# RaikoPipe/panda-gym

Hardware: AMD Instinct MI355X
Metric: aggregate env-steps/s, PandaReach 4096 envs @1 GPU; 1/2/4/8-GPU scaling (higher is better)
Workload: dtype f32; 1 GPU; PandaReach-v3 (ee control, sparse reward), 4096 envs per GPU, the reference's scene: table / plane contacts of the robot (BASELINE configs[1]); envs_per_gpu=4096, global_envs=4096, parallelism=env-sharded x1

## Files before the change

panda-gym_amd/csrc/pgx_api.cpp:

```cpp
#include <hip/hip_runtime.h>

#include <cmath>
#include <cstdarg>
#include <cstdio>
#include <cstdlib>
#include <cstring>
#include <string>
#include <vector>

#include "../../include/pgx.h"
#include "pgx_default_model.h"
#include "pgx_dev.h"
#include "pgx_model_consts.h"
#include "pgx_rows.h"

namespace {

thread_local std::string g_err;

int fail(int code, const char* fmt, ...) __attribute__((format(printf, 2, 3)));
int fail(int code, const char* fmt, ...) {
    char buf[512];
    va_list ap;
    va_start(ap, fmt);
// ... 10 lines not shown

void m3mul(const double* A, const double* B, double* C) {
    double t[9];
    for (int i = 0; i < 3; i++)
        for (int j = 0; j < 3; j++) t[i * 3 + j] = A[i * 3] * B[j] + A[i * 3 + 1] * B[3 + j] + A[i * 3 + 2] * B[6 + j];
    std::memcpy(C, t, sizeof t);
}
void m3v(const double* A, const double* v, double* o) {
    double t[3];
    for (int i = 0; i < 3; i++) t[i] = A[i * 3] * v[0] + A[i * 3 + 1] * v[1] + A[i * 3 + 2] * v[2];
    std::memcpy(o, t, sizeof t);
}

}

int pgx_set_error(int code, const char* msg) {
    g_err = msg;
    return code;
}

struct pgx_env {
    int device;
    PgxDevModel dm;
    PgxDevModel* dm_dev;
    PgxDevEnv de;
    PgxDevState ds;
    void* blob;
    size_t blob_bytes;
    std::vector<void*> snaps;
    uint64_t* pcg = nullptr;
    bool pcg_set = false;
    int man_pool = 0;
    const char* step_kernel = nullptr;
};

extern "C" {

const char* pgx_version(void) { return "pgx 0.1.0 (gfx950)"; }
const char* pgx_last_error(void) { return g_err.c_str(); }

int pgx_obs_dim(const pgx_config* c) {
    if (!c) return PGX_E_INVALID;
    if (c->task == PGX_TASK_REACH_AO) return 20 + 4 * PGX_AO_LINKS;
    return 6 + (c->block_gripper ? 0 : 1) + (c->task == PGX_TASK_REACH ? 0 : 12);
}
int pgx_action_dim(const pgx_config* c) {
    if (!c) return PGX_E_INVALID;
    return (c->control == PGX_CONTROL_EE ? 3 : 7) + (c->block_gripper ? 0 : 1);
}

static int check_compiled_tables(const PgxDevModel& dm) {
    auto same = [](const float* a, const float* b, int n, const char* what) -> int {
        for (int i = 0; i < n; i++)
            if (std::fabs(a[i] - b[i]) > 1e-6f * std::fmax(1.0f, std::fabs(b[i])))
                return fail(PGX_E_UNSUPPORTED, "model table %s[%d] = %g differs from the compiled robot (%g)", what,
                            i, (double)a[i], (double)b[i]);
        return PGX_OK;
    };
    int rc = 0;
    rc = rc ? rc : same(&dm.jp[0][0], &kJp[0][0], 21, "jp");
    rc = rc ? rc : same(&dm.jr[0][0], &kJr[0][0], 63, "jr");
    rc = rc ? rc : same(&dm.com[0][0], &kCom[0][0], 21, "com");
    rc = rc ? rc : same(dm.mass, kMass, 7, "mass");
    rc = rc ? rc : same(&dm.inertia[0][0], &kInertia[0][0], 18, "inertia");
    rc = rc ? rc : same(dm.i6c, kI6c, 6, "i6c");
    rc = rc ? rc : same(dm.i6own, kI6own, 6, "i6own");
// ... 294 lines not shown
        return fail(PGX_E_INVALID, "n_substeps must be in [1, 1000], got %d", cfg->params->n_substeps);
    pgx_env* h = new pgx_env();
    h->device = device;
    int rc = build_dev_model(cfg, &h->dm);
    if (rc) { delete h; return rc; }
#ifndef PGX_RUNTIME_MODEL
    {
        static_assert(sizeof(PgxDevModel) == 4 * PGX_DEV_MODEL_WORDS, "default model block size");
        const PgxDevModelWords& def = cfg->task == PGX_TASK_REACH_AO ? kDefModelAoWords : kDefModelArmWords;
        uint32_t got[PGX_DEV_MODEL_WORDS];
        std::memcpy(got, &h->dm, sizeof got);
        for (int i = 0; i < PGX_DEV_MODEL_WORDS; i++)
            if (got[i] != def.w[i]) {
                delete h;
                return fail(PGX_E_UNSUPPORTED,
                            "physics / robot parameters differ from the ones the kernels are compiled for "
                            "(constant block word %d: 0x%08x, compiled 0x%08x; tools/gen_default_model.py)",
                            i, got[i], def.w[i]);
            }
    }
#endif
    PgxDevEnv& e = h->de;
    e.pcg = nullptr;
    e.pcg_on = nullptr;
    e.perm_buf = nullptr;
    e.perm = nullptr;
    e.sort_mode = 0;
    if (const char* so = std::getenv("PGX_SORT_ENVS")) e.sort_mode = std::atoi(so) ? 1 : -1;
    e.sort_key = 1;
    if (const char* sk = std::getenv("PGX_SORT_KEY")) e.sort_key = std::atoi(sk) ? 1 : 0;
    e.sort_segs = 0;
    if (const char* sg = std::getenv("PGX_SORT_SEGS")) e.sort_segs = std::atoi(sg) == 1 ? 1 : 0;
    e.perm_segs = 1;
    e.task = cfg->task;
    e.control = cfg->control;
    e.reward = cfg->reward;
    e.n_envs = cfg->n_envs;
    e.max_episode_steps = cfg->max_episode_steps;
    e.block_gripper = cfg->block_gripper;
    e.obs_dim = pgx_obs_dim(cfg);
    e.action_dim = pgx_action_dim(cfg);
    e.seed = cfg->seed;
    e.env_id_offset = cfg->env_id_offset;
    e.distance_threshold = cfg->distance_threshold;
    for (int c = 0; c < 3; c++) { e.goal_low[c] = cfg->goal_low[c]; e.goal_high[c] = cfg->goal_high[c]; }
    for (int c = 0; c < 3; c++) {
        e.goal_offset[c] = cfg->goal_offset[c];
        e.obj_low[c] = cfg->obj_low[c];
        e.obj_high[c] = cfg->obj_high[c];
        e.obj_offset[c] = cfg->obj_offset[c];
    }
    e.goal_z_zero_prob = cfg->goal_z_zero_prob;
    e.contacts = cfg->contacts ? 1 : 0;
    e.full_manifold = cfg->contacts == PGX_CONTACTS_FULL ? 1 : 0;
    e.has_object = has_object;
    e.obj_half = (float)cfg->object_half;
    e.obj_inv_mass = e.has_object ? (float)(1.0 / cfg->object_mass) : 0.0f;
    e.obj_inv_inertia = e.has_object ? (float)(1.0 / cfg->object_inertia) : 0.0f;
    e.table_cx = (float)cfg->table_center[0];
    e.table_cy = (float)cfg->table_center[1];
    e.table_hx = (float)cfg->table_half[0];
    e.table_hy = (float)cfg->table_half[1];
    e.table_top = (float)(cfg->table_center[2] + cfg->table_half[2]);
    e.plane_z = (float)cfg->plane_z;
    e.table_hz = (float)cfg->table_half[2];
    e.ao = cfg->task == PGX_TASK_REACH_AO;
// ... 9 lines not shown
    }
    e.pgs_mode = 0;
    if (const char* pm = std::getenv("PGX_PGS_MODE")) e.pgs_mode = std::atoi(pm);
    e.n_substeps = cfg->params->n_substeps;
    e.wave_mode = 0;
    if (const char* wm = std::getenv("PGX_WAVES_PER_SIMD")) e.wave_mode = std::atoi(wm);
    const int wide_max = 8192;
    e.lanes_per_env = cfg->lanes_per_env ? cfg->lanes_per_env
                                         : ((cfg->n_envs <= wide_max || cfg->contacts) ? 16 : 1);
    if (const char* lpe = std::getenv("PGX_LANES_PER_ENV")) {
        const int v = std::atoi(lpe);
        if (v != 1 && v != 16) { delete h; return fail(PGX_E_INVALID, "PGX_LANES_PER_ENV must be 1 or 16, got %s", lpe); }
        e.lanes_per_env = v;
    }
    if (e.full_manifold && e.lanes_per_env != 16) {
        delete h;
        return fail(PGX_E_UNSUPPORTED, "PGX_CONTACTS_FULL needs the 16-lane layout (the one-lane kernels keep 4 robot points)");
    }

    rc = hip_check(hipSetDevice(device), "hipSetDevice");
    if (rc) { delete h; return rc; }
    const size_t N = (size_t)cfg->n_envs;
    auto align = [](size_t x) { return (x + 255) & ~(size_t)255; };
    const int man_pool = (e.full_manifold && (e.has_object || e.ao)) ? (e.has_object ? PGX_MANIFOLD_POOL
                                                                                     : PGX_MANIFOLD_POOL_AO) : 0;
    const size_t man_rows = man_pool ? 1 + (size_t)man_pool * PGX_MANIFOLD_POINT : 0;
    h->man_pool = man_pool;
    size_t off_goal = align(sizeof(PgxDevModel)), off_q = align(off_goal + 3 * N * 8), off_qd = align(off_q + PGX_NJ * N * 4),
           off_qc = align(off_qd + PGX_NJ * N * 4), off_obj = align(off_qc + PGX_NJ * N * 4), off_ct = align(off_obj + 13 * N * 4),
           off_ao = align(off_ct + 2 * PGX_CONTACT_SLOTS * N * 4),
           off_man = align(off_ao + (e.ao ? 4 * PGX_AO_OBSTACLES * N * 4 : 0)),
           off_el = align(off_man + man_rows * N * 4), off_ep = align(off_el + N * 4),
           off_err = align(off_ep + N * 4), off_perm = align(off_err + 4),
           total = align(off_perm + (e.full_manifold ? N * 4 + (N + 3) / 4 * 4 + (N / 256 + 1) * 13 * 4 : 0));
    rc = hip_check(hipMalloc(&h->blob, total), "hipMalloc(state)");
    if (rc) { delete h; return rc; }
    h->blob_bytes = total;
    char* b = (char*)h->blob;
    h->ds.goal = (double*)(b + off_goal);
    h->ds.q = (float*)(b + off_q);
    h->ds.qd = (float*)(b + off_qd);
    h->ds.qc = (float*)(b + off_qc);
    h->ds.object = (float*)(b + off_obj);
    h->ds.contacts = (float*)(b + off_ct);
    h->ds.obstacles = e.ao ? (float*)(b + off_ao) : nullptr;
    h->ds.man = man_pool ? (float*)(b + off_man) : nullptr;
    h->ds.elapsed = (int32_t*)(b + off_el);
    h->ds.episode = (uint32_t*)(b + off_ep);
    h->ds.errors = (uint32_t*)(b + off_err);
    if (e.full_manifold) e.perm_buf = (int32_t*)(b + off_perm);
    h->dm_dev = (PgxDevModel*)b;
    const size_t pcg_bytes = align(8 * PGX_PCG64_WORDS * N);
    const size_t geo_bytes = e.ao ? align(8 * PGX_AO_GEO_DOUBLES) : 0;
    rc = hip_check(hipMalloc((void**)&h->pcg, pcg_bytes + 256 + geo_bytes), "hipMalloc(rng streams)");
    if (rc) { h->pcg = nullptr; (void)hipFree(h->blob); delete h; return rc; }
    e.pcg = h->pcg;
    e.pcg_on = (const int32_t*)((char*)h->pcg + pcg_bytes);
    e.ao_geo = e.ao ? (const double*)((char*)h->pcg + pcg_bytes + 256) : nullptr;
    rc = hip_check(hipMemset(h->pcg, 0, pcg_bytes + 256), "hipMemset(rng streams)");
    if (!rc && e.ao) {
        double geo[PGX_AO_GEO_DOUBLES];
        ao_reset_geometry(cfg, geo);
        rc = hip_check(hipMemcpy((void*)e.ao_geo, geo, sizeof geo, hipMemcpyHostToDevice), "ReachAO geometry copy");
    }
    if (!rc) rc = hip_check(hipMemset(h->blob, 0, total), "hipMemset(state)");
    if (!rc) rc = hip_check(hipMemcpy(h->dm_dev, &h->dm, sizeof(PgxDevModel), hipMemcpyHostToDevice), "model copy");
    if (!rc && e.perm_buf) {
        std::vector<int32_t> ident(N);
        for (size_t k = 0; k < N; k++) ident[k] = (int32_t)k;
        rc = hip_check(hipMemcpy(e.perm_buf, ident.data(), N * 4, hipMemcpyHostToDevice), "env order init");
    }
    if (!rc) {
        PgxDevOut none;
        std::memset(&none, 0, sizeof none);
        rc = hip_check((hipError_t)pgx_launch_reset(h->dm_dev, h->de, h->ds, nullptr, nullptr, nullptr, none, nullptr),
                       "reset launch");
        if (!rc) rc = hip_check(hipMemset(h->ds.episode, 0, N * 4), "hipMemset(episode)");
        if (!rc) rc = hip_check(hipDeviceSynchronize(), "create sync");
    }
    if (rc) { (void)hipFree(h->pcg); (void)hipFree(h->blob); delete h; return rc; }
    *out = h;
    return PGX_OK;
}
// ... 22 lines not shown
    out->errors = h->ds.errors;
    out->robot_points = !h->de.contacts ? 0
                      : !h->de.full_manifold ? PGX_ROBOT_POINTS_ONE_LANE
                      : h->de.has_object ? PGX_ROBOT_POINTS : PGX_ROBOT_POINTS_ARM;
    out->env_order = h->de.perm_buf;
    out->manifolds = h->ds.man;
    out->manifold_pool = h->man_pool;
    return PGX_OK;
}

static PgxDevOut to_dev_out(const pgx_step_out* o) {
    PgxDevOut d;
    std::memset(&d, 0, sizeof d);
    if (!o) return d;
    d.obs = o->obs;
    d.ag = o->achieved_goal;
    d.dg = o->desired_goal;
    d.reward = o->reward;
    d.success = o->success;
    d.terminated = o->terminated;
    d.truncated = o->truncated;
    d.terminal_obs = o->terminal_obs;
    d.terminal_ag = o->terminal_achieved_goal;
    d.terminal_dg = o->terminal_desired_goal;
    d.task_truncated = o->task_truncated;
    return d;
}

int pgx_reset(pgx_handle h, const uint8_t* env_mask, const double* inject_goal, const double* inject_object,
              pgx_step_out* out, void* stream) {
    if (!h) return fail(PGX_E_INVALID, "null handle");
    if (inject_object && !h->de.has_object && !h->de.ao)
        return fail(PGX_E_INVALID, "object injection needs an object task (or ReachAO obstacles)");
    return hip_check((hipError_t)pgx_launch_reset(h->dm_dev, h->de, h->ds, env_mask, inject_goal, inject_object,
                                                  to_dev_out(out), stream),
                     "reset launch");
}

int pgx_step(pgx_handle h, const float* action, pgx_step_out* out, void* stream) {
    if (!h || !action) return fail(PGX_E_INVALID, "null argument");
    if (out && out->nonfinite && !h->de.nonfinite_guard) {
        const int rc = hip_check((hipError_t)pgx_launch_zero_flags(out->nonfinite, h->de.n_envs, stream), "flags launch");
        if (rc) return rc;
    }
    return hip_check((hipError_t)pgx_launch_step(h->dm_dev, h->de, h->ds, action, to_dev_out(out), stream,
                                                 &h->step_kernel, out ? out->nonfinite : nullptr),
                     "step launch");
}

const char* pgx_step_kernel(pgx_handle h) { return h ? h->step_kernel : nullptr; }

int pgx_sample_actions(pgx_handle h, float* action, uint64_t step, void* stream) {
    if (!h || !action) return fail(PGX_E_INVALID, "null argument");
    return hip_check((hipError_t)pgx_launch_sample_actions(h->de, action, step, stream), "sample launch");
}

int pgx_compute_reward(const float* ag, const float* dg, int64_t batch, int32_t reward_type, double thr, float* out,
                       void* stream) {
    if (batch < 0 || (batch > 0 && (!ag || !dg || !out))) return fail(PGX_E_INVALID, "bad arguments");
    if (reward_type != PGX_REWARD_SPARSE && reward_type != PGX_REWARD_DENSE && reward_type != PGX_REWARD_SPARSE_AO)
        return fail(PGX_E_INVALID, "reward_type %d", reward_type);
    return hip_check((hipError_t)pgx_launch_compute_reward(ag, dg, batch, reward_type, thr, out, stream),
                     "compute_reward launch");
}

int pgx_state_bytes(pgx_handle h, int64_t* nbytes) {
    if (!h || !nbytes) return fail(PGX_E_INVALID, "null argument");
    *nbytes = (int64_t)h->blob_bytes;
    return PGX_OK;
}

int pgx_save_state(pgx_handle h, void* dst, void* stream) {
    if (!h || !dst) return fail(PGX_E_INVALID, "null argument");
    return hip_check(hipMemcpyAsync(dst, h->blob, h->blob_bytes, hipMemcpyDeviceToDevice, (hipStream_t)stream),
                     "save_state copy");
}

int pgx_restore_state(pgx_handle h, const void* src, void* stream) {
    if (!h || !src) return fail(PGX_E_INVALID, "null argument");
    return hip_check(hipMemcpyAsync(h->blob, src, h->blob_bytes, hipMemcpyDeviceToDevice, (hipStream_t)stream),
                     "restore_state copy");
}

int pgx_snapshot(pgx_handle h, int32_t* state_id, void* stream) {
    if (!h || !state_id) return fail(PGX_E_INVALID, "null argument");
    *state_id = -1;
    size_t id = 0;
    while (id < h->snaps.size() && h->snaps[id]) id++;
    int rc = hip_check(hipSetDevice(h->device), "hipSetDevice");
    void* buf = nullptr;
    if (!rc) rc = hip_check(hipMalloc(&buf, h->blob_bytes), "hipMalloc(snapshot)");
    if (rc) return rc;
    rc = hip_check(hipMemcpyAsync(buf, h->blob, h->blob_bytes, hipMemcpyDeviceToDevice, (hipStream_t)stream),
                   "snapshot copy");
    if (rc) { (void)hipFree(buf); return rc; }
    if (id == h->snaps.size()) h->snaps.push_back(buf);
    else h->snaps[id] = buf;
    *state_id = (int32_t)id;
    return PGX_OK;
}

static bool snap_valid(pgx_handle h, int32_t id) {
    return id >= 0 && (size_t)id < h->snaps.size() && h->snaps[id] != nullptr;
}

int pgx_restore(pgx_handle h, int32_t state_id, void* stream) {
    if (!h) return fail(PGX_E_INVALID, "null handle");
    if (!snap_valid(h, state_id)) return fail(PGX_E_INVALID, "Couldn't restore state %d: no such saved state", state_id);
    return hip_check(hipMemcpyAsync(h->blob, h->snaps[state_id], h->blob_bytes, hipMemcpyDeviceToDevice,
                                    (hipStream_t)stream),
                     "restore copy");
}

int pgx_release(pgx_handle h, int32_t state_id) {
    if (!h) return fail(PGX_E_INVALID, "null handle");
    if (!snap_valid(h, state_id)) return fail(PGX_E_INVALID, "Couldn't remove state %d: no such saved state", state_id);
    int rc = hip_check(hipSetDevice(h->device), "hipSetDevice");
    if (!rc) rc = hip_check(hipDeviceSynchronize(), "release sync");
    if (!rc) rc = hip_check(hipFree(h->snaps[state_id]), "hipFree(snapshot)");
    h->snaps[state_id] = nullptr;
    return rc;
}

int pgx_set_rng_streams(pgx_handle h, const uint64_t* states, void* stream) {
    if (!h) return fail(PGX_E_INVALID, "null handle");
    int rc = hip_check(hipSetDevice(h->device), "hipSetDevice");
    if (rc) return rc;
    int32_t* on = const_cast<int32_t*>(h->de.pcg_on);
    if (states)
        rc = hip_check(hipMemcpyAsync(h->pcg, states, 8 * PGX_PCG64_WORDS * (size_t)h->de.n_envs, hipMemcpyDefault, (hipStream_t)stream),
                       "rng streams copy");
    if (!rc) rc = hip_check((hipError_t)pgx_launch_set_word(on, states ? 1 : 0, stream), "rng mode word");
    if (!rc) h->pcg_set = states != nullptr;
    return rc;
}

int pgx_get_rng_streams(pgx_handle h, uint64_t* states, void* stream) {
    if (!h || !states) return fail(PGX_E_INVALID, "null argument");
    if (!h->pcg_set) return fail(PGX_E_INVALID, "no PCG64 reset streams set (pgx_set_rng_streams)");
    return hip_check(hipMemcpyAsync(states, h->pcg, 8 * PGX_PCG64_WORDS * (size_t)h->de.n_envs, hipMemcpyDefault, (hipStream_t)stream),
                     "rng streams copy");
// ... 4 lines not shown
```

panda-gym_amd/csrc/pgx_dev.h:

```cpp
#pragma once
#include <stdint.h>

#define PGX_NJ 7
#define PGX_MAX_DAMP 4

struct PgxDevModel {
    float jp[PGX_NJ][3];
    float jr[PGX_NJ][9];
    float com[PGX_NJ][3];
    float mass[PGX_NJ];
    float inertia[PGX_NJ - 1][3];
    float i6c[6];
    float i6own[6];
    float dpos[PGX_MAX_DAMP][3];
    float dmass[PGX_MAX_DAMP];
    int32_t ndamp;
    float ee_pivot[3];
    float ee_rot[9];
    float ee_com[3];
    float lower[PGX_NJ], upper[PGX_NJ];
    float max_impulse[PGX_NJ];
    float dt, inv_dt;
    float gravity[3];
    float lin_damp, ang_damp, max_vel, residual_thr, erp, limit_max_imp, kp, kd;
// ... 13 lines not shown
struct PgxDevEnv {
    int32_t task, control, reward, n_envs;
    int32_t max_episode_steps, block_gripper, obs_dim, action_dim;
    uint64_t seed, env_id_offset;
    double distance_threshold;
    double goal_low[3], goal_high[3];
    double goal_offset[3], goal_z_zero_prob;
    double obj_low[3], obj_high[3], obj_offset[3];
    int32_t contacts, has_object;
    float obj_half, obj_inv_mass, obj_inv_inertia;
    float table_cx, table_cy, table_hx, table_hy, table_top, plane_z;
    float table_hz;
    int32_t ao;
    int32_t terminate_on_success;
    int32_t no_auto_reset;
    double collision_reward;
    double ao_ee[3];
    int32_t ao_ee_set;
    const double* ao_geo;
    int32_t lanes_per_env;
    int32_t pgs_mode;
    int32_t n_substeps;
    int32_t full_manifold;
    int32_t wave_mode;
    uint64_t* pcg;
    const int32_t* pcg_on;
    int32_t* perm_buf;
    int32_t sort_mode;
    int32_t sort_key;
    int32_t sort_segs;
    const int32_t* perm;
    int32_t perm_segs;
    int32_t nonfinite_guard;
};

struct PgxDevState {
    float* q;
    float* qd;
    float* qc;
    double* goal;
    float* object;
    float* contacts;
    float* obstacles;
    float* man;
    int32_t* elapsed;
    uint32_t* episode;
    uint32_t* errors;
};

struct PgxDevOut {
    float* obs;
    float* ag;
    float* dg;
    float* reward;
    uint8_t* success;
    uint8_t* terminated;
    uint8_t* truncated;
    float* terminal_obs;
    float* terminal_ag;
    float* terminal_dg;
    uint8_t* task_truncated;
};

int pgx_launch_step_arm(const PgxDevModel* m_device, const PgxDevEnv& e, const PgxDevState& s, const float* action,
                        const PgxDevOut& o, void* stream, const char** name, uint8_t* nonfinite);
int pgx_launch_step(const PgxDevModel* m_device, const PgxDevEnv& e, const PgxDevState& s, const float* action,
// ... 17 lines not shown
```

panda-gym_amd/csrc/pgx_kernels.hip:

```cpp
#include <hip/hip_runtime.h>
#include <math.h>
#include <stdint.h>

#include "../../include/pgx.h"
#include "pgx_default_model.h"
#include "pgx_common.h"
#include "pgx_dev.h"
#include "pgx_model_consts.h"
#include "pgx_rows.h"

#ifdef PGX_PROF
#define PGX_PROF_N 24
__device__ unsigned long long pgx_prof_counters[PGX_PROF_N];
#define PGX_PROF_WAVES 16384
__device__ unsigned long long pgx_prof_wave[PGX_PROF_WAVES][10];
extern "C" int pgx_prof_wave_read(unsigned long long* out, int n) {
    return (int)hipMemcpyFromSymbol(out, HIP_SYMBOL(pgx_prof_wave), sizeof(unsigned long long) * 10 * (size_t)n);
}
extern "C" int pgx_prof_read(unsigned long long* out, int clear) {
    hipError_t e = hipMemcpyFromSymbol(out, HIP_SYMBOL(pgx_prof_counters), sizeof(unsigned long long) * PGX_PROF_N);
    if (e == hipSuccess && clear) {
        unsigned long long z[PGX_PROF_N] = {0};
        e = hipMemcpyToSymbol(HIP_SYMBOL(pgx_prof_counters), z, sizeof z);
    }
// ... 3895 lines not shown
        if (t < AO_N - n_active) { L.aoC[pt][0][ln] = 99.9f; L.aoC[pt][1][ln] = 99.9f; L.aoC[pt][2][ln] = -99.9f; }
    }
    if (inject_goal) { goal[0] = inject_goal[0]; goal[1] = inject_goal[1]; goal[2] = inject_goal[2]; }
    if (inject_obst)
        for (int o = 0; o < AO_N; o++)
            for (int k = 0; k < 3; k++) L.aoC[o][k][ln] = (float)inject_obst[3 * o + k];
    if (rec && lead && !inject_goal && !inject_obst) pcg64_store(d.g, rec);
    return failed && !inject_obst;
}

template <class LT>
__device__ __forceinline__ void ao_load(const PgxDevState& s, int N, int i, LT& L, int ln) {
#pragma unroll
    for (int o = 0; o < AO_N; o++)
#pragma unroll
        for (int k = 0; k < 3; k++) L.aoC[o][k][ln] = s.obstacles[(3 * o + k) * N + i];
}
template <class LT>
__device__ __forceinline__ void ao_store(const PgxDevState& s, int N, int i, const LT& L, int ln) {
#pragma unroll
    for (int o = 0; o < AO_N; o++) {
#pragma unroll
        for (int k = 0; k < 3; k++) s.obstacles[(3 * o + k) * N + i] = L.aoC[o][k][ln];
        s.obstacles[(3 * AO_N + o) * N + i] = L.aoC[o][0][ln] < 50.0f ? 1.0f : 0.0f;
    }
}

__device__ __forceinline__ int xcd_block() {
    const int nb = gridDim.x, b = blockIdx.x;
    if (nb % 8) return b;
    return (b % 8) * (nb / 8) + b / 8;
}

template <int CONTROL, int OBJ, int CONT, int AO, int WIDE, int PART = 1, int GUARD = 0>
__device__ __forceinline__ void step_body(const PgxDevModel* __restrict__ mdev, const PgxDevEnv& e,
                                          const PgxDevState& s, const float* __restrict__ action, const PgxDevOut& o,
                                          uint8_t* nf_out = nullptr) {
    constexpr int FULL = WIDE == 2 ? 1 : 0;
    using LT = ContactLdsT<WIDE ? EPW : 64, WIDE ? OBJ : 1, FULL>;
    constexpr int CACHE_K = 2 * (CG + LT::RB);
    const int ln = WIDE ? (int)threadIdx.x / GW : (int)threadIdx.x;
    const int c = WIDE ? (int)threadIdx.x % GW : 0;
    const bool lead = c == 0;
    const int N = e.n_envs;
    const int slot = ((e.perm && e.perm_segs == 1) ? (int)blockIdx.x : xcd_block()) * (WIDE ? EPW : 64) + ln;
    if (slot >= N) return;
    const int i = e.perm ? e.perm[slot] : slot;
#ifdef PGX_CHECK_PERM
    if ((unsigned)i >= (unsigned)N) {
        printf("pgx: perm[%d] = %d outside [0, %d)\n", slot, i, N);
        __builtin_trap();
    }
#endif
    int ii = i;
    asm volatile("" : "+v"(ii));
    LT* L = nullptr;
    if constexpr (CONT) {
        __shared__ LT lds_buf;
        L = &lds_buf;
#ifdef PGX_LDS_POISON
        {
            float* w = reinterpret_cast<float*>(L);
            for (size_t t = threadIdx.x; t < sizeof(LT) / 4; t += blockDim.x) w[t] = __builtin_nanf("");
            __syncthreads();
        }
#endif
#pragma unroll
        for (int k = 0; k < (WIDE ? 0 : CG); k++) {
#pragma unroll
            for (int qq = 0; qq < 4; qq++) L->g0q[k][qq][ln] = make_float4(0.0f, 0.0f, 0.0f, 0.0f);
            L->g0n[k][0][ln] = 0.0f; L->g0n[k][1][ln] = 0.0f; L->g0n[k][2][ln] = 1.0f;
#pragma unroll
            for (int dir = 0; dir < 3; dir++)
#pragma unroll
                for (int qq = 0; qq < 6; qq++) L->g1q[k][dir][qq][ln] = make_float4(0.0f, 0.0f, 0.0f, 0.0f);
        }
    }
#ifdef PGX_PROF
    if (threadIdx.x < PGX_PROF_N) g_prof[threadIdx.x] = 0;
    g_prof_t = __builtin_amdgcn_s_memtime();
// ... 106 lines not shown
            if constexpr (AO) asm volatile("" : "+v"(cl), "+v"(esl));
            if (substep_g<OBJ, CONT, PART, AO, FULL>(mp, e, q, qd, tq, ob, L, esl, cl, lk, AO && st > 0)) {
                collided = true;
                break;
            }
        } else {
            substep<OBJ, CONT, AO>(mp, e, q, qd, tq, ob, L, ln);
        }
        if constexpr (PARK) qslot = st & 1;
        else {
#pragma unroll
            for (int j = 0; j < NJ; j++) qprev[j] = qstart[j];
        }
        if constexpr (AO && !WIDE) {
            ao_caps(*fresh(mp), q, *L, ln);
            if (ao_collided(e, *L, ln)) { collided = true; break; }
        }
    }
    if constexpr (AO && WIDE) {
        if (!collided) {
            ao_caps(*fresh(mp), q, *L, ln);
            collided = ao_collided_g(e, *L, ln, c);
        }
    }

    if constexpr (PARK) {
#pragma unroll
        for (int j = 0; j < NJ; j++) qprev[j] = lds_ld(&L->lqs[qslot][j][ln]);
    }
    int ie = i;
    if constexpr (AO) {
        int lnx = ln;
        asm volatile("" : "+v"(lnx));
        const int sl = ((e.perm && e.perm_segs == 1) ? (int)blockIdx.x : xcd_block()) * (WIDE ? EPW : 64) + lnx;
        ie = e.perm ? __hip_atomic_load(&e.perm[sl], __ATOMIC_RELAXED, __HIP_MEMORY_SCOPE_AGENT) : sl;
    }
    double goal[3];
#pragma unroll
    for (int c = 0; c < 3; c++) goal[c] = s.goal[c * N + (AO ? ie : ii)];
    V3 pos, vel;
    ee_state_cached(*fresh(mp), qprev, q, qd, pos, vel);
#ifdef PGX_NAN_TRAP
    if constexpr (!WIDE) {
        const float pv[6] = {pos.x, pos.y, pos.z, vel.x, vel.y, vel.z};
        PGX_TRAP(7, 0, pv, 6, m);
    }
#endif
    const int od = e.obs_dim;
    const V3 ag = OBJ ? ob.p : pos;
    double d = distance_f32_f64(ag, goal);
    bool succ = d < e.distance_threshold;
    float rew;
    if (AO) {
        rew = -1.0f + ((d + (collided ? 1.0 : 0.0)) < e.distance_threshold ? 1.0f : 0.0f);
        if (collided) rew += (float)e.collision_reward;
    } else {
        rew = e.reward == 0 ? -((d > e.distance_threshold) ? 1.0f : 0.0f) : -(float)d;
    }
    int el = s.elapsed[ie] + 1;
    uint32_t episode = s.episode[ie];
    bool trunc = (e.max_episode_steps > 0 && el >= e.max_episode_steps) || collided;
    bool term = e.terminate_on_success && succ;
    bool bad = false;
    if constexpr (GUARD) {
        if constexpr (AO) {
            if constexpr (WIDE) ao_link_obs_g(*L, ln, c);
            else ao_link_obs(*L, ln);
// ... 105 lines not shown
    if (o.dg) {
        o.dg[3 * (size_t)ie] = (float)goal[0]; o.dg[3 * (size_t)ie + 1] = (float)goal[1];
        o.dg[3 * (size_t)ie + 2] = (float)goal[2];
    }
    if constexpr (GUARD) {
        if (bad && !e.no_auto_reset) {
            if (o.terminal_obs) {
                if constexpr (AO) ao_write_obs(o.terminal_obs + (size_t)ie * od, pos, vel, q, qd, *L, ln);
                else write_obs<OBJ>(e, o.terminal_obs + (size_t)ie * od, pos, vel, ob);
            }
            if (o.terminal_ag) {
                o.terminal_ag[3 * (size_t)ie] = ag2.x; o.terminal_ag[3 * (size_t)ie + 1] = ag2.y;
                o.terminal_ag[3 * (size_t)ie + 2] = ag2.z;
            }
            if (o.terminal_dg) {
                o.terminal_dg[3 * (size_t)ie] = (float)goal[0]; o.terminal_dg[3 * (size_t)ie + 1] = (float)goal[1];
                o.terminal_dg[3 * (size_t)ie + 2] = (float)goal[2];
            }
        }
    }
#pragma unroll
    for (int j = 0; j < NJ; j++) {
        s.q[j * N + ie] = q[j];
        s.qd[j * N + ie] = qd[j];
        s.qc[j * N + ie] = qprev[j];
    }
#pragma unroll
    for (int c = 0; c < 3; c++) s.goal[c * N + ie] = goal[c];
    if (OBJ) store_obj(s, N, ie, ob);
    if constexpr (AO) ao_store(s, N, ie, *L, ln);
    if (CONT) {
#pragma unroll
        for (int k = 0; k < CACHE_K; k++) s.contacts[k * N + ie] = L->cache[k][ln];
    }
    s.elapsed[ie] = el;
    s.episode[ie] = episode;
#ifdef PGX_PROF
    PGX_PROF_MARK(6);
    if (threadIdx.x == 0) {
        for (int k = 0; k < PGX_PROF_N; k++) atomicAdd(&pgx_prof_counters[k], g_prof[k]);
        if (blockIdx.x < PGX_PROF_WAVES) {
            unsigned long long* w = pgx_prof_wave[blockIdx.x];
            w[0] = prof_t0; w[1] = g_prof_t; w[2] = g_prof[8]; w[3] = g_prof[10]; w[4] = g_prof[12]; w[5] = g_prof[13];
            w[6] = g_prof[7]; w[7] = g_prof[4]; w[8] = g_prof[1]; w[9] = g_prof[6];
        }
    }
#endif
}

template <int AO>
__device__ __forceinline__ void scene_from_model(PgxDevEnv& e, const PgxDevModel* mdev) {
    if constexpr (!AO) return;
    MRef m = *model_ptr<AO>(mdev);
    e.table_cx = m.table_cx; e.table_cy = m.table_cy; e.table_hx = m.table_hx; e.table_hy = m.table_hy;
    e.table_top = m.table_top; e.plane_z = m.plane_z; e.table_hz = m.table_hz;
}
template <int CONTROL, int OBJ, int CONT, int AO, int WIDE>
__global__ __launch_bounds__(64) void step_kernel(const PgxDevModel* __restrict__ mdev, PgxDevEnv e, PgxDevState s,
                                                  const float* __restrict__ action, PgxDevOut o) {
    scene_from_model<AO>(e, mdev);
    step_body<CONTROL, OBJ, CONT, AO, WIDE>(mdev, e, s, action, o);
}
template <int CONTROL, int OBJ, int CONT, int AO, int WIDE>
__global__ __launch_bounds__(64) __attribute__((amdgpu_waves_per_eu(2, 2))) void step_kernel_o2(
    const PgxDevModel* __restrict__ mdev, PgxDevEnv e, PgxDevState s, const float* __restrict__ action, PgxDevOut o) {
    scene_from_model<AO>(e, mdev);
// ... 80 lines not shown
    if (OBJ) store_obj(s, N, i, ob);
    if constexpr (AO) ao_store(s, N, i, *L, ln);
#pragma unroll
    for (int k = 0; k < CACHE_N; k++) s.contacts[k * N + i] = (k & 1) ? 0.0f : -1.0f;
    if (s.man) s.man[i] = 0.0f;
    s.elapsed[i] = 0;
    s.episode[i] = episode;
}

__global__ __launch_bounds__(256) void sample_actions_kernel(PgxDevEnv e, float* action, uint64_t step) {
    const int i = blockIdx.x * blockDim.x + threadIdx.x;
    if (i >= e.n_envs) return;
    const int A = e.action_dim;
    const uint64_t env = e.env_id_offset + (uint64_t)i;
    uint32_t o[4];
    for (int a = 0; a < A; a++) {
        if ((a & 3) == 0)
            philox((uint32_t)env, (uint32_t)(env >> 32), (uint32_t)step,
                   TAG_ACTION + ((uint32_t)(step >> 32) << 4) + (uint32_t)(a >> 2), (uint32_t)e.seed,
                   (uint32_t)(e.seed >> 32), o);
        uint32_t u = o[a & 3];
        action[(size_t)i * A + a] = (float)(u >> 8) * (1.0f / 16777216.0f) * 2.0f - 1.0f;
    }
}

__global__ __launch_bounds__(256) void compute_reward_kernel(const float* __restrict__ ag, const float* __restrict__ dg,
                                                             int64_t n, int32_t reward_type, float thr,
                                                             float* __restrict__ out) {
    for (int64_t i = blockIdx.x * (int64_t)blockDim.x + threadIdx.x; i < n; i += (int64_t)gridDim.x * blockDim.x) {
        out[i] = reward_f32(distance_f32_f32(ag + 3 * i, dg + 3 * i), reward_type, thr);
    }
}

constexpr int SORT_BINS = PGX_ROBOT_POINTS + 1;
constexpr int SORT_BLOCK = 256;
__global__ __launch_bounds__(SORT_BLOCK) void env_sort_keys_kernel(PgxDevState s, int N, int rb, int all, uint8_t* keys,
                                                                   int32_t* blk) {
    __shared__ int32_t wc[SORT_BLOCK / 64][SORT_BINS];
    const int i = blockIdx.x * SORT_BLOCK + threadIdx.x, lane = (int)__lane_id(), w = (int)threadIdx.x / 64;
    int key = -1;
    if (i < N) {
        key = 0;
        for (int r = 0; r < rb; r++) key += s.contacts[(size_t)(CACHE1 + 2 * r) * N + i] >= 0.0f ? 1 : 0;
        if (!all) key = key > CG ? key - CG : 0;
        keys[i] = (uint8_t)key;
    }
    for (int k = 0; k < SORT_BINS; k++) {
        const int c = __popcll(__ballot(key == k));
        if (lane == 0) wc[w][k] = c;
    }
    __syncthreads();
    if (threadIdx.x < SORT_BINS) {
        int c = 0;
        for (int ww = 0; ww < SORT_BLOCK / 64; ww++) c += wc[ww][threadIdx.x];
        blk[(size_t)blockIdx.x * SORT_BINS + threadIdx.x] = c;
    }
}
__global__ __launch_bounds__(SORT_BLOCK) void env_sort_scatter_kernel(int N, const uint8_t* keys, const int32_t* blk,
                                                                      int32_t* perm, int segs) {
    __shared__ int32_t base[SORT_BINS];
    __shared__ int32_t wc[SORT_BLOCK / 64][SORT_BINS];
    const int bps = (int)gridDim.x / segs, me = (int)blockIdx.x, sg = me / bps;
    const int b0 = sg * bps, nb = b0 + bps;
    const int i = me * SORT_BLOCK + threadIdx.x, lane = (int)__lane_id(), w = (int)threadIdx.x / 64;
    __shared__ int32_t red[SORT_BLOCK / 64][2][SORT_BINS];
    int tot[SORT_BINS], pre[SORT_BINS];
#pragma unroll
// ... 9 lines not shown
#pragma unroll
    for (int k = 0; k < SORT_BINS; k++) {
#pragma unroll
        for (int d = 32; d >= 1; d >>= 1) {
            tot[k] += __shfl_xor(tot[k], d);
            pre[k] += __shfl_xor(pre[k], d);
        }
        if (lane == 0) { red[w][0][k] = tot[k]; red[w][1][k] = pre[k]; }
    }
    __syncthreads();
    if (threadIdx.x < SORT_BINS) {
        const int k = threadIdx.x;
        int off = 0;
        for (int kk = SORT_BINS - 1; kk > k; kk--)
            for (int ww = 0; ww < SORT_BLOCK / 64; ww++) off += red[ww][0][kk];
        for (int ww = 0; ww < SORT_BLOCK / 64; ww++) off += red[ww][1][k];
        base[k] = off + sg * (N / segs);
    }
    const int key = i < N ? (int)keys[i] : -1;
    uint64_t mine_k = 0ull;
    for (int k = 0; k < SORT_BINS; k++) {
        const uint64_t m = __ballot(key == k);
        if (key == k) mine_k = m;
        if (lane == 0) wc[w][k] = __popcll(m);
    }
    __syncthreads();
    if (key >= 0) {
        int r = base[key] + __popcll(mine_k & ((1ull << lane) - 1ull));
        for (int ww = 0; ww < w; ww++) r += wc[ww][key];
        perm[r] = i;
    }
}

constexpr int SORT_SEG_MAX = 1024;
__global__ __launch_bounds__(SORT_SEG_MAX) void env_sort_segment_kernel(PgxDevState s, int N, int rb, int all,
                                                                        int32_t* perm) {
    __shared__ int32_t wc[SORT_SEG_MAX / 64][SORT_BINS];
    __shared__ int32_t base[SORT_BINS];
    const int S = (int)blockDim.x, t = (int)threadIdx.x, lane = (int)__lane_id(), w = t / 64, nw = (S + 63) / 64;
    const int i = (int)blockIdx.x * S + t;
    int key = 0;
    for (int r = 0; r < rb; r++) key += s.contacts[(size_t)(CACHE1 + 2 * r) * N + i] >= 0.0f ? 1 : 0;
    if (!all) key = key > CG ? key - CG : 0;
    uint64_t mine_k = 0ull;
    for (int k = 0; k < SORT_BINS; k++) {
        const uint64_t m = __ballot(key == k);
        if (key == k) mine_k = m;
        if (lane == 0) wc[w][k] = __popcll(m);
    }
    __syncthreads();
    if (t < SORT_BINS) {
        int off = 0;
        for (int kk = SORT_BINS - 1; kk > t; kk--)
            for (int ww = 0; ww < nw; ww++) off += wc[ww][kk];
        base[t] = off;
    }
    __syncthreads();
    int r = base[key] + __popcll(mine_k & ((1ull << lane) - 1ull));
    for (int ww = 0; ww < w; ww++) r += wc[ww][key];
    perm[(int)blockIdx.x * S + r] = i;
}

}

#ifndef PGX_TU
#define PGX_TU 0
#endif
// ... 13 lines not shown
        if (two) {                                                                                           \
            hipLaunchKernelGGL((step_kernel_o2_nf<C, O, K, A, W>), grid, block, 0, st, m, e, s, action, o, nf); \
            if (name) *name = PGX_KNAME(step_kernel_o2_nf, C, O, K, A, W);                                   \
        } else {                                                                                             \
            PGX_STEP(C, O, K, A, W);                                                                         \
        }                                                                                                    \
    } while (0)
#else
#define PGX_FN(f) f
#define PGX_STEP(C, O, K, A, W)                                                                   \
    do {                                                                                          \
        hipLaunchKernelGGL((step_kernel<C, O, K, A, W>), grid, block, 0, st, m, e, s, action, o); \
        if (name) *name = PGX_KNAME(step_kernel, C, O, K, A, W);                                  \
    } while (0)
#define PGX_STEP2(C, O, K, A, W)                                                                      \
    do {                                                                                              \
        if (two) {                                                                                    \
            hipLaunchKernelGGL((step_kernel_o2<C, O, K, A, W>), grid, block, 0, st, m, e, s, action, o); \
            if (name) *name = PGX_KNAME(step_kernel_o2, C, O, K, A, W);                                \
        } else {                                                                                      \
            PGX_STEP(C, O, K, A, W);                                                                  \
        }                                                                                             \
    } while (0)
#endif
#if PGX_TU != 3 && PGX_TU != 4
constexpr unsigned kSortMinWaves = 256u;
static PgxDevEnv sort_envs(const PgxDevEnv& e, const PgxDevState& s, hipStream_t st) {
    PgxDevEnv es = e;
    const int rb = e.has_object ? PGX_ROBOT_POINTS : PGX_ROBOT_POINTS_ARM;
    {
        const int segs = (e.sort_segs != 1 && e.n_envs % (8 * SORT_BLOCK) == 0) ? 8 : 1;
        const int S = e.n_envs / segs;
        if (S <= SORT_SEG_MAX && S > 0) {
            hipLaunchKernelGGL(env_sort_segment_kernel, dim3(segs), dim3(S), 0, st, s, e.n_envs, rb, e.sort_key,
                               e.perm_buf);
            es.perm = e.perm_buf;
            es.perm_segs = segs;
            return es;
        }
    }
    const int nb = (e.n_envs + SORT_BLOCK - 1) / SORT_BLOCK;
    uint8_t* keys = reinterpret_cast<uint8_t*>(e.perm_buf + e.n_envs);
    int32_t* blk = e.perm_buf + e.n_envs + (e.n_envs + 3) / 4;
    hipLaunchKernelGGL(env_sort_keys_kernel, dim3(nb), dim3(SORT_BLOCK), 0, st, s, e.n_envs, rb, e.sort_key, keys, blk);
    const int segs = (e.sort_segs != 1 && e.n_envs % (8 * SORT_BLOCK) == 0) ? 8 : 1;
    hipLaunchKernelGGL(env_sort_scatter_kernel, dim3(nb), dim3(SORT_BLOCK), 0, st, e.n_envs, (const uint8_t*)keys,
                       (const int32_t*)blk, e.perm_buf, segs);
    es.perm = e.perm_buf;
    es.perm_segs = segs;
    return es;
}
#endif
#if PGX_TU == 4 || PGX_TU == 0
int PGX_FN(pgx_launch_step_ao)(const PgxDevModel* m, const PgxDevEnv& e, const PgxDevState& s, const float* action,
                               const PgxDevOut& o, void* stream, const char** name, bool two, bool wide, uint8_t* nf) {
    hipStream_t st = (hipStream_t)stream;
    const int per_block = wide ? EPW : 64;
    dim3 block(64), grid((e.n_envs + per_block - 1) / per_block);
    if (wide && e.full_manifold) PGX_STEP2(1, 0, 1, 1, 2);
    else if (wide) PGX_STEP2(1, 0, 1, 1, 1);
    else PGX_STEP(1, 0, 1, 1, 0);
    return (int)hipGetLastError();
}
#endif
#if PGX_TU != 2 && PGX_TU != 3 && PGX_TU != 4
int PGX_FN(pgx_launch_step_arm)(const PgxDevModel* m, const PgxDevEnv& e, const PgxDevState& s, const float* action,
                                const PgxDevOut& o, void* stream, const char** name, uint8_t* nf) {
    hipStream_t st = (hipStream_t)stream;
    const int wide = e.lanes_per_env == GW;
    const int per_block = wide ? EPW : 64;
    dim3 block(64), grid((e.n_envs + per_block - 1) / per_block);
    const bool two = e.wave_mode == 2 || (e.wave_mode == 0 && wide && grid.x > 1024);
    if (wide && e.contacts && e.full_manifold) {
        PgxDevEnv es = e;
        es.perm = nullptr;
        if (e.perm_buf && (e.sort_mode == 1 || (e.sort_mode == 0 && grid.x >= kSortMinWaves))) es = sort_envs(e, s, st);
        const PgxDevEnv& e = es;
        if (e.control) PGX_STEP(1, 0, 1, 0, 2);
        else PGX_STEP2(0, 0, 1, 0, 2);
        return (int)hipGetLastError();
    }
    switch ((e.control * 4 + (e.contacts ? 1 : 0)) * 2 + wide) {
        case 0: PGX_STEP(0, 0, 0, 0, 0); break;
        case 1: PGX_STEP(0, 0, 0, 0, 1); break;
        case 2: PGX_STEP(0, 0, 1, 0, 0); break;
        case 3: PGX_STEP2(0, 0, 1, 0, 1); break;
        case 8: PGX_STEP(1, 0, 0, 0, 0); break;
        case 9: PGX_STEP(1, 0, 0, 0, 1); break;
        case 10: PGX_STEP(1, 0, 1, 0, 0); break;
        case 11: PGX_STEP(1, 0, 1, 0, 1); break;
        default: return (int)hipErrorInvalidValue;
    }
    return (int)hipGetLastError();
}
#endif
#if PGX_TU != 1 && PGX_TU != 3 && PGX_TU != 4
int PGX_FN(pgx_launch_step)(const PgxDevModel* m, const PgxDevEnv& e, const PgxDevState& s, const float* action,
                             const PgxDevOut& o, void* stream, const char** name, uint8_t* nf) {
#if !PGX_NF
    if (e.nonfinite_guard) {
#if PGX_TU == 0 || defined(PGX_NO_NF)
        return (int)hipErrorNotSupported;
#else
        return pgx_launch_step_nf(m, e, s, action, o, stream, name, nf);
#endif
    }
#endif
    if (!e.ao && !e.has_object) return PGX_FN(pgx_launch_step_arm)(m, e, s, action, o, stream, name, nf);
    hipStream_t st = (hipStream_t)stream;
    const int wide = e.lanes_per_env == GW;
    const int per_block = wide ? EPW : 64;
    dim3 block(64), grid((e.n_envs + per_block - 1) / per_block);
    const bool two = e.wave_mode == 2 || (e.wave_mode == 0 && wide && grid.x > 1024);
    const int variant = e.control * 4 + (e.has_object ? 2 : 0) + (e.contacts ? 1 : 0);
    if (wide && e.full_manifold) {
        const bool sort = e.perm_buf && (e.sort_mode == 1 || (e.sort_mode == 0 && grid.x >= kSortMinWaves));
        PgxDevEnv es = e;
        es.perm = nullptr;
        if (sort) es = sort_envs(e, s, st);
        const PgxDevEnv& e = es;
        if (e.ao) return PGX_FN(pgx_launch_step_ao)(m, e, s, action, o, stream, name, two, true, nf);
        switch (variant) {
            case 3: PGX_STEP(0, 1, 1, 0, 2); break;
            case 7: PGX_STEP(1, 1, 1, 0, 2); break;
            default: return (int)hipErrorInvalidValue;
        }
        return (int)hipGetLastError();
    }
    if (e.ao) return PGX_FN(pgx_launch_step_ao)(m, e, s, action, o, stream, name, two, wide, nf);
    switch (variant * 2 + wide) {
        case 6: PGX_STEP(0, 1, 1, 0, 0); break;
        case 7: PGX_STEP2(0, 1, 1, 0, 1); break;
        case 14: PGX_STEP(1, 1, 1, 0, 0); break;
        case 15: PGX_STEP2(1, 1, 1, 0, 1); break;
        default: return (int)hipErrorInvalidValue;
    }
    return (int)hipGetLastError();
}

#if !PGX_NF
int pgx_launch_reset(const PgxDevModel* m, const PgxDevEnv& e, const PgxDevState& s, const uint8_t* mask,
                     const double* inject_goal, const double* inject_obj, const PgxDevOut& o, void* stream) {
    dim3 block(64), grid((e.n_envs + 63) / 64);
    if (e.ao)
        hipLaunchKernelGGL((reset_kernel<0, 1>), grid, block, 0, (hipStream_t)stream, m, e, s, mask, inject_goal, inject_obj, o);
    else if (e.has_object)
        hipLaunchKernelGGL((reset_kernel<1, 0>), grid, block, 0, (hipStream_t)stream, m, e, s, mask, inject_goal, inject_obj, o);
    else
        hipLaunchKernelGGL((reset_kernel<0, 0>), grid, block, 0, (hipStream_t)stream, m, e, s, mask, inject_goal, inject_obj, o);
    return (int)hipGetLastError();
}
// ... 37 lines not shown
```

Before: 11.63 million env-steps/s.

## Fuse env contact-sort ordering into the step kernel using previous-step keys

The step kernel now writes each env's contact-count sort key into a double-buffered key array. On the next step, every wave rebuilds its own slice of the sorted permutation in-register: it reads the segment's keys, binary-searches the key bucket, and uses DPP prefix sums and ballots to pick the env for each slot. This replaces the separate segment-sort kernel launch. In exchange, every wave does redundant selection work over the whole segment, and the ordering uses keys one step old. A host-side reference model of the ordering is added, and an env var can turn the fused path off.

```diff
diff --git a/panda-gym_amd/csrc/pgx_api.cpp b/panda-gym_amd/csrc/pgx_api.cpp
--- a/panda-gym_amd/csrc/pgx_api.cpp
+++ b/panda-gym_amd/csrc/pgx_api.cpp
@@ -66,6 +66,10 @@
     bool pcg_set = false;
     int man_pool = 0;
     const char* step_kernel = nullptr;
+    uint8_t* key_buf[2] = {nullptr, nullptr};
+    int key_write = 0;
+    bool keys_fresh = false;
+    bool sort_fused = true;
 };
 
 extern "C" {
@@ -426,6 +430,9 @@
     e.sort_segs = 0;
     if (const char* sg = std::getenv("PGX_SORT_SEGS")) e.sort_segs = std::atoi(sg) == 1 ? 1 : 0;
     e.perm_segs = 1;
+    e.keys_in = nullptr;
+    e.keys_out = nullptr;
+    if (const char* sf = std::getenv("PGX_SORT_FUSED")) h->sort_fused = std::atoi(sf) != 0;
     e.task = cfg->task;
     e.control = cfg->control;
     e.reward = cfg->reward;
@@ -501,7 +508,9 @@
            off_man = align(off_ao + (e.ao ? 4 * PGX_AO_OBSTACLES * N * 4 : 0)),
            off_el = align(off_man + man_rows * N * 4), off_ep = align(off_el + N * 4),
            off_err = align(off_ep + N * 4), off_perm = align(off_err + 4),
-           total = align(off_perm + (e.full_manifold ? N * 4 + (N + 3) / 4 * 4 + (N / 256 + 1) * 13 * 4 : 0));
+           off_keys = off_perm + ((e.full_manifold ? N * 4 + (N + 3) / 4 * 4 + (N / 256 + 1) * 13 * 4 : 0) + 15) / 16 * 16,
+           key_bytes = (N + 15) / 16 * 16,
+           total = align(off_keys + (e.full_manifold ? 2 * key_bytes : 0));
     rc = hip_check(hipMalloc(&h->blob, total), "hipMalloc(state)");
     if (rc) { delete h; return rc; }
     h->blob_bytes = total;
@@ -517,7 +526,11 @@
     h->ds.elapsed = (int32_t*)(b + off_el);
     h->ds.episode = (uint32_t*)(b + off_ep);
     h->ds.errors = (uint32_t*)(b + off_err);
-    if (e.full_manifold) e.perm_buf = (int32_t*)(b + off_perm);
+    if (e.full_manifold) {
+        e.perm_buf = (int32_t*)(b + off_perm);
+        h->key_buf[0] = (uint8_t*)(b + off_keys);
+        h->key_buf[1] = (uint8_t*)(b + off_keys + key_bytes);
+    }
     h->dm_dev = (PgxDevModel*)b;
     const size_t pcg_bytes = align(8 * PGX_PCG64_WORDS * N);
     const size_t geo_bytes = e.ao ? align(8 * PGX_AO_GEO_DOUBLES) : 0;
@@ -606,6 +619,7 @@
     if (!h) return fail(PGX_E_INVALID, "null handle");
     if (inject_object && !h->de.has_object && !h->de.ao)
         return fail(PGX_E_INVALID, "object injection needs an object task (or ReachAO obstacles)");
+    h->keys_fresh = false;
     return hip_check((hipError_t)pgx_launch_reset(h->dm_dev, h->de, h->ds, env_mask, inject_goal, inject_object,
                                                   to_dev_out(out), stream),
                      "reset launch");
@@ -617,9 +631,18 @@
         const int rc = hip_check((hipError_t)pgx_launch_zero_flags(out->nonfinite, h->de.n_envs, stream), "flags launch");
         if (rc) return rc;
     }
-    return hip_check((hipError_t)pgx_launch_step(h->dm_dev, h->de, h->ds, action, to_dev_out(out), stream,
-                                                 &h->step_kernel, out ? out->nonfinite : nullptr),
-                     "step launch");
+    if (h->de.perm_buf) {
+        h->de.keys_out = h->key_buf[h->key_write];
+        h->de.keys_in = (h->sort_fused && h->keys_fresh) ? h->key_buf[h->key_write ^ 1] : nullptr;
+    }
+    const int rc = hip_check((hipError_t)pgx_launch_step(h->dm_dev, h->de, h->ds, action, to_dev_out(out), stream,
+                                                         &h->step_kernel, out ? out->nonfinite : nullptr),
+                             "step launch");
+    if (h->de.perm_buf) {
+        h->key_write ^= 1;
+        h->keys_fresh = rc == PGX_OK;
+    }
+    return rc;
 }
 
 const char* pgx_step_kernel(pgx_handle h) { return h ? h->step_kernel : nullptr; }
@@ -652,6 +675,7 @@
 
 int pgx_restore_state(pgx_handle h, const void* src, void* stream) {
     if (!h || !src) return fail(PGX_E_INVALID, "null argument");
+    h->keys_fresh = false;
     return hip_check(hipMemcpyAsync(h->blob, src, h->blob_bytes, hipMemcpyDeviceToDevice, (hipStream_t)stream),
                      "restore_state copy");
 }
@@ -681,6 +705,7 @@
 int pgx_restore(pgx_handle h, int32_t state_id, void* stream) {
     if (!h) return fail(PGX_E_INVALID, "null handle");
     if (!snap_valid(h, state_id)) return fail(PGX_E_INVALID, "Couldn't restore state %d: no such saved state", state_id);
+    h->keys_fresh = false;
     return hip_check(hipMemcpyAsync(h->blob, h->snaps[state_id], h->blob_bytes, hipMemcpyDeviceToDevice,
                                     (hipStream_t)stream),
                      "restore copy");
diff --git a/panda-gym_amd/csrc/pgx_dev.h b/panda-gym_amd/csrc/pgx_dev.h
--- a/panda-gym_amd/csrc/pgx_dev.h
+++ b/panda-gym_amd/csrc/pgx_dev.h
@@ -69,6 +69,8 @@
     const int32_t* perm;
     int32_t perm_segs;
     int32_t nonfinite_guard;
+    const uint8_t* keys_in;
+    uint8_t* keys_out;
 };
 
 struct PgxDevState {
diff --git a/panda-gym_amd/csrc/pgx_kernels.hip b/panda-gym_amd/csrc/pgx_kernels.hip
--- a/panda-gym_amd/csrc/pgx_kernels.hip
+++ b/panda-gym_amd/csrc/pgx_kernels.hip
@@ -3951,6 +3951,104 @@
     return (b % 8) * (nb / 8) + b / 8;
 }
 
+__device__ __forceinline__ int env_block(const PgxDevEnv& e) {
+    return (e.perm && e.perm_segs == 1) ? (int)blockIdx.x : xcd_block();
+}
+
+constexpr int SORT_BINS = PGX_ROBOT_POINTS + 1;
+constexpr int SORT_SEG_MAX = 1024;
+constexpr int ORDER_KPL = SORT_SEG_MAX / 64;
+static_assert(ORDER_KPL == GW && EPW * GW == 64, "the pick inside the lane: one lane of the env's row per key");
+template <int CTRL, int ROWS>
+__device__ __forceinline__ int dpp_add0(int x) {
+    return x + __builtin_amdgcn_update_dpp(0, x, CTRL, ROWS, 0xF, false);
+}
+__device__ __forceinline__ int wave_prefix_sum(int x) {
+    x = dpp_add0<0x111, 0xF>(x);
+    x = dpp_add0<0x112, 0xF>(x);
+    x = dpp_add0<0x114, 0xF>(x);
+    x = dpp_add0<0x118, 0xF>(x);
+    x = dpp_add0<0x142, 0xA>(x);
+    x = dpp_add0<0x143, 0xC>(x);
+    return x;
+}
+template <int TOP>
+__device__ __forceinline__ int order_env(const uint8_t* __restrict__ keys, int N, int segs, int ln) {
+    const int lane = (int)threadIdx.x;
+    const int S = segs == 1 ? N : N >> 3;
+    const int base = segs == 1 ? 0 : (int)(blockIdx.x & 7u) * S;
+    const int r0 = (segs == 1 ? (int)blockIdx.x : (int)(blockIdx.x >> 3)) * EPW;
+    const int nv = S - ORDER_KPL * lane;
+    uint32_t kw[4] = {0u, 0u, 0u, 0u};
+    if (nv > 0) {
+        const uint4 v = *reinterpret_cast<const uint4*>(keys + base + ORDER_KPL * lane);
+        kw[0] = v.x; kw[1] = v.y; kw[2] = v.z; kw[3] = v.w;
+    }
+    if (S & (ORDER_KPL - 1)) {
+#pragma unroll
+        for (int d = 0; d < 4; d++) {
+            const int nd = nv - 4 * d;
+            kw[d] &= nd <= 0 ? 0u : 0x7f7f7f7fu >> (32 - 8 * min(nd, 4));
+        }
+    } else {
+#pragma unroll
+        for (int d = 0; d < 4; d++) kw[d] &= 0x7f7f7f7fu;
+    }
+    int lo = 0, hi = TOP, B = 0;
+    while (lo < hi) {
+        const int mid = (lo + hi + 1) >> 1;
+        const uint32_t up = 0x01010101u * (uint32_t)(0x80 - mid);
+        int c = 0;
+#pragma unroll
+        for (int d = 0; d < 4; d++) c += __popc((kw[d] + up) & 0x80808080u);
+        const int g = __builtin_amdgcn_readlane(wave_prefix_sum(c), 63);
+        if (g > r0) {
+            lo = mid;
+        } else {
+            hi = mid - 1;
+            B = g;
+        }
+    }
+    int lsel = 0, jsel = 0, ksel = 0xff;
+    for (int k = lo; k >= 0; k--) {
+        const uint32_t kk = 0x01010101u * (uint32_t)k;
+        int nz = 0;
+#pragma unroll
+        for (int d = 0; d < 4; d++) nz += __popc(((kw[d] ^ kk) + 0x7f7f7f7fu) & 0x80808080u);
+        const int c = ORDER_KPL - nz;
+        const int x = wave_prefix_sum(c);
+        const int T = __builtin_amdgcn_readlane(x, 63);
+        const int p0 = r0 - B;
+        if (p0 < T && p0 + EPW > 0) {
+            const int E = x - c;
+#pragma unroll
+            for (int t = 0; t < EPW; t++) {
+                const int p = p0 + t;
+                if (p >= 0 && p < T) {
+                    const int lt = min((int)__popcll(__ballot(x <= p)), 63);
+                    const int j = p - __builtin_amdgcn_readlane(E, lt);
+                    if (ln == t) { lsel = lt; jsel = j; ksel = k; }
+                }
+            }
+        }
+        B += T;
+        if (B >= r0 + EPW) break;
+    }
+    const int b = lane & (ORDER_KPL - 1);
+    uint32_t w = (uint32_t)__shfl((int)kw[0], lsel);
+    const uint32_t w1 = (uint32_t)__shfl((int)kw[1], lsel), w2 = (uint32_t)__shfl((int)kw[2], lsel),
+                   w3 = (uint32_t)__shfl((int)kw[3], lsel);
+    w = (b >> 2) == 1 ? w1 : w;
+    w = (b >> 2) == 2 ? w2 : w;
+    w = (b >> 2) == 3 ? w3 : w;
+    const bool match = (int)((w >> (8 * (b & 3))) & 0xffu) == ksel;
+    const uint32_t gm = (uint32_t)(__ballot(match) >> (ORDER_KPL * ln)) & 0xffffu;
+    const bool hit = match && __popc(gm & ((1u << b) - 1u)) == jsel;
+    const uint32_t gh = (uint32_t)(__ballot(hit) >> (ORDER_KPL * ln)) & 0xffffu;
+    const int i = base + ORDER_KPL * lsel + (int)__builtin_ctz(gh | 0x10000u);
+    return min(max(i, base), base + S - 1);
+}
+
 template <int CONTROL, int OBJ, int CONT, int AO, int WIDE, int PART = 1, int GUARD = 0>
 __device__ __forceinline__ void step_body(const PgxDevModel* __restrict__ mdev, const PgxDevEnv& e,
                                           const PgxDevState& s, const float* __restrict__ action, const PgxDevOut& o,
@@ -3962,9 +4060,21 @@
     const int c = WIDE ? (int)threadIdx.x % GW : 0;
     const bool lead = c == 0;
     const int N = e.n_envs;
-    const int slot = ((e.perm && e.perm_segs == 1) ? (int)blockIdx.x : xcd_block()) * (WIDE ? EPW : 64) + ln;
+    const int slot = env_block(e) * (WIDE ? EPW : 64) + ln;
+    bool keyed = false;
+    int ikey = 0;
+    if constexpr (WIDE == 2) {
+        keyed = e.keys_in != nullptr;
+        if (keyed) ikey = order_env<LT::RB>(e.keys_in, N, e.perm_segs, ln);
+    }
     if (slot >= N) return;
-    const int i = e.perm ? e.perm[slot] : slot;
+    int i;
+    if (keyed) {
+        i = ikey;
+        e.perm_buf[slot] = i;
+    } else {
+        i = e.perm ? e.perm[slot] : slot;
+    }
 #ifdef PGX_CHECK_PERM
     if ((unsigned)i >= (unsigned)N) {
         printf("pgx: perm[%d] = %d outside [0, %d)\n", slot, i, N);
@@ -4137,7 +4247,7 @@
     if constexpr (AO) {
         int lnx = ln;
         asm volatile("" : "+v"(lnx));
-        const int sl = ((e.perm && e.perm_segs == 1) ? (int)blockIdx.x : xcd_block()) * (WIDE ? EPW : 64) + lnx;
+        const int sl = env_block(e) * (WIDE ? EPW : 64) + lnx;
         ie = e.perm ? __hip_atomic_load(&e.perm[sl], __ATOMIC_RELAXED, __HIP_MEMORY_SCOPE_AGENT) : sl;
     }
     double goal[3];
@@ -4309,6 +4419,15 @@
     if (CONT) {
 #pragma unroll
         for (int k = 0; k < CACHE_K; k++) s.contacts[k * N + ie] = L->cache[k][ln];
+    }
+    if constexpr (WIDE == 2 && CONT) {
+        if (e.keys_out) {
+            int key = 0;
+#pragma unroll
+            for (int r = 0; r < LT::RB; r++) key += L->cache[CACHE1 + 2 * r][ln] >= 0.0f ? 1 : 0;
+            if (!e.sort_key) key = key > CG ? key - CG : 0;
+            e.keys_out[ie] = (uint8_t)key;
+        }
     }
     s.elapsed[ie] = el;
     s.episode[ie] = episode;
@@ -4455,7 +4574,6 @@
     }
 }
 
-constexpr int SORT_BINS = PGX_ROBOT_POINTS + 1;
 constexpr int SORT_BLOCK = 256;
 __global__ __launch_bounds__(SORT_BLOCK) void env_sort_keys_kernel(PgxDevState s, int N, int rb, int all, uint8_t* keys,
                                                                    int32_t* blk) {
@@ -4531,7 +4649,6 @@
     }
 }
 
-constexpr int SORT_SEG_MAX = 1024;
 __global__ __launch_bounds__(SORT_SEG_MAX) void env_sort_segment_kernel(PgxDevState s, int N, int rb, int all,
                                                                         int32_t* perm) {
     __shared__ int32_t wc[SORT_SEG_MAX / 64][SORT_BINS];
@@ -4611,13 +4728,15 @@
         const int segs = (e.sort_segs != 1 && e.n_envs % (8 * SORT_BLOCK) == 0) ? 8 : 1;
         const int S = e.n_envs / segs;
         if (S <= SORT_SEG_MAX && S > 0) {
-            hipLaunchKernelGGL(env_sort_segment_kernel, dim3(segs), dim3(S), 0, st, s, e.n_envs, rb, e.sort_key,
-                               e.perm_buf);
             es.perm = e.perm_buf;
             es.perm_segs = segs;
+            if (!e.keys_in)
+                hipLaunchKernelGGL(env_sort_segment_kernel, dim3(segs), dim3(S), 0, st, s, e.n_envs, rb, e.sort_key,
+                                   e.perm_buf);
             return es;
         }
     }
+    es.keys_in = nullptr;
     const int nb = (e.n_envs + SORT_BLOCK - 1) / SORT_BLOCK;
     uint8_t* keys = reinterpret_cast<uint8_t*>(e.perm_buf + e.n_envs);
     int32_t* blk = e.perm_buf + e.n_envs + (e.n_envs + 3) / 4;
@@ -4653,6 +4772,7 @@
     if (wide && e.contacts && e.full_manifold) {
         PgxDevEnv es = e;
         es.perm = nullptr;
+        es.keys_in = nullptr;
         if (e.perm_buf && (e.sort_mode == 1 || (e.sort_mode == 0 && grid.x >= kSortMinWaves))) es = sort_envs(e, s, st);
         const PgxDevEnv& e = es;
         if (e.control) PGX_STEP(1, 0, 1, 0, 2);
@@ -4696,6 +4816,7 @@
         const bool sort = e.perm_buf && (e.sort_mode == 1 || (e.sort_mode == 0 && grid.x >= kSortMinWaves));
         PgxDevEnv es = e;
         es.perm = nullptr;
+        es.keys_in = nullptr;
         if (sort) es = sort_envs(e, s, st);
         const PgxDevEnv& e = es;
         if (e.ao) return PGX_FN(pgx_launch_step_ao)(m, e, s, action, o, stream, name, two, true, nf);
diff --git a/panda-gym_amd/csrc/pgx_order_model.cpp b/panda-gym_amd/csrc/pgx_order_model.cpp
--- /dev/null
+++ b/panda-gym_amd/csrc/pgx_order_model.cpp
@@ -0,0 +1,124 @@
+#include <stdint.h>
+#include <string.h>
+
+namespace {
+constexpr int WAVE = 64, GW = 16, EPW = WAVE / GW, KPL = 16;
+
+int popc(uint32_t x) { return __builtin_popcount(x); }
+
+void row_shr_add(int* x, int n) {
+    int y[WAVE];
+    for (int l = 0; l < WAVE; l++) y[l] = x[l] + ((l % 16) >= n ? x[l - n] : 0);
+    memcpy(x, y, sizeof y);
+}
+void row_bcast_add(int* x, int which, unsigned rows) {
+    int y[WAVE];
+    for (int l = 0; l < WAVE; l++) {
+        const int row = l / 16;
+        const int src = which == 15 ? row * 16 - 1 : 31;
+        y[l] = x[l] + (((rows >> row) & 1u) && src >= 0 ? x[src] : 0);
+    }
+    memcpy(x, y, sizeof y);
+}
+void wave_prefix_sum(int* x) {
+    row_shr_add(x, 1);
+    row_shr_add(x, 2);
+    row_shr_add(x, 4);
+    row_shr_add(x, 8);
+    row_bcast_add(x, 15, 0xA);
+    row_bcast_add(x, 31, 0xC);
+}
+uint64_t ballot(const bool* p) {
+    uint64_t m = 0;
+    for (int l = 0; l < WAVE; l++) m |= (uint64_t)p[l] << l;
+    return m;
+}
+}
+
+extern "C" void pgx_order_model(const uint8_t* keys, int N, int segs, int block, int top, int32_t* out) {
+    const int S = segs == 1 ? N : N >> 3;
+    const int base = segs == 1 ? 0 : (block & 7) * S;
+    const int r0 = (segs == 1 ? block : block >> 3) * EPW;
+    uint32_t kw[4][WAVE];
+    for (int l = 0; l < WAVE; l++) {
+        const int nv = S - KPL * l;
+        for (int d = 0; d < 4; d++) kw[d][l] = 0u;
+        if (nv > 0) {
+            for (int d = 0; d < 4; d++) memcpy(&kw[d][l], keys + base + KPL * l + 4 * d, 4);
+        }
+        for (int d = 0; d < 4; d++) {
+            const int nd = nv - 4 * d;
+            kw[d][l] &= nd <= 0 ? 0u : 0x7f7f7f7fu >> (32 - 8 * (nd > 4 ? 4 : nd));
+        }
+    }
+    int lo = 0, hi = top, B = 0;
+    while (lo < hi) {
+        const int mid = (lo + hi + 1) >> 1;
+        const uint32_t up = 0x01010101u * (uint32_t)(0x80 - mid);
+        int x[WAVE];
+        for (int l = 0; l < WAVE; l++) {
+            x[l] = 0;
+            for (int d = 0; d < 4; d++) x[l] += popc((kw[d][l] + up) & 0x80808080u);
+        }
+        wave_prefix_sum(x);
+        const int g = x[63];
+        if (g > r0) {
+            lo = mid;
+        } else {
+            hi = mid - 1;
+            B = g;
+        }
+    }
+    int lsel[WAVE], jsel[WAVE], ksel[WAVE];
+    for (int l = 0; l < WAVE; l++) { lsel[l] = 0; jsel[l] = 0; ksel[l] = 0xff; }
+    for (int k = lo; k >= 0; k--) {
+        const uint32_t kk = 0x01010101u * (uint32_t)k;
+        int c[WAVE], x[WAVE];
+        for (int l = 0; l < WAVE; l++) {
+            int nz = 0;
+            for (int d = 0; d < 4; d++) nz += popc(((kw[d][l] ^ kk) + 0x7f7f7f7fu) & 0x80808080u);
+            c[l] = KPL - nz;
+            x[l] = c[l];
+        }
+        wave_prefix_sum(x);
+        const int T = x[63];
+        const int p0 = r0 - B;
+        if (p0 < T && p0 + EPW > 0) {
+            for (int t = 0; t < EPW; t++) {
+                const int p = p0 + t;
+                if (p >= 0 && p < T) {
+                    bool in[WAVE];
+                    for (int l = 0; l < WAVE; l++) in[l] = x[l] <= p;
+                    int lt = __builtin_popcountll(ballot(in));
+                    lt = lt > 63 ? 63 : lt;
+                    const int j = p - (x[lt] - c[lt]);
+                    for (int l = 0; l < WAVE; l++)
+                        if (l / GW == t) { lsel[l] = lt; jsel[l] = j; ksel[l] = k; }
+                }
+            }
+        }
+        B += T;
+        if (B >= r0 + EPW) break;
+    }
+    bool match[WAVE], hit[WAVE];
+    for (int l = 0; l < WAVE; l++) {
+        const int b = l & (KPL - 1);
+        const uint32_t w = kw[b >> 2][lsel[l]];
+        match[l] = (int)((w >> (8 * (b & 3))) & 0xffu) == ksel[l];
+    }
+    const uint64_t mm = ballot(match);
+    for (int l = 0; l < WAVE; l++) {
+        const int b = l & (KPL - 1), ln = l / GW;
+        const uint32_t gm = (uint32_t)(mm >> (KPL * ln)) & 0xffffu;
+        hit[l] = match[l] && popc(gm & ((1u << b) - 1u)) == jsel[l];
+    }
+    const uint64_t hm = ballot(hit);
+    for (int t = 0; t < EPW; t++) {
+        const int l = t * GW;
+        const uint32_t gh = (uint32_t)(hm >> (KPL * t)) & 0xffffu;
+        int i = base + KPL * lsel[l] + __builtin_ctz(gh | 0x10000u);
+        i = i < base ? base : i;
+        i = i > base + S - 1 ? base + S - 1 : i;
+        out[t] = i;
+    }
+}
```

Result: faster. 11.75 million env-steps/s (median of 6 runs) (+1.0%).
